# CILAB-MA/gpudrive_lab

Hardware: AMD Instinct MI355X
Metric: agent-steps/sec at 1024 worlds x 64 agents; achieved HBM GB/s on obs kernel (higher is better)
Workload: dtype f32

## Files before the change

gpudrive_lab_amd/csrc/engine.cpp:

```cpp
#include <hip/hip_runtime.h>

#include <algorithm>
#include <cmath>
#include <cstdlib>
#include <cstdio>
#include <cstring>
#include <map>
#include <memory>
#include <stdexcept>
#include <atomic>
#include <exception>
#include <string>
#include <thread>
#include <vector>

#include "dev_mem.hpp"
#include "engine.hpp"
#include "gd_math.hpp"
#include "scene.hpp"
#ifdef GD_CLOCKS
namespace gd { void set_clocks_read(unsigned long long *out); void step_clocks_read(unsigned long long *out); }
#endif
#ifndef GD_GRID_MIN_CELL
#define GD_GRID_MIN_CELL 16.f
// ... 125 lines not shown
    std::vector<gd::DevMem> internal;
    std::vector<std::string> scenes;
    std::vector<int32_t> deleted;
    std::vector<WorldHost> world_host;
    int cu_count = 256;
    Growable<float2, 320, 640> road_xy;
    Growable<Float8, 320, 640> road_aux, road_rec;
    Growable<gd::RoadBox, 0, 64> boxes;
    Growable<int32_t, 0, 64> cell_off, cell_items;
    Growable<float4, 0, 64> cell_hdr;
    Growable<int32_t, 0, 64> rcell_off;
    Growable<uint16_t, 64, 128> rcell_items, rcell_pos;
    Growable<float2, 64, 128> rcell_xy;
    Growable<float4, 0, 64> road_blk;
    int32_t *d_road_off = nullptr, *d_box_off = nullptr, *d_blk_off = nullptr;
    gd::GridHdr *d_grid = nullptr, *d_rgrid = nullptr;
    float4 *d_road_bbox = nullptr;
    float *d_road_rbmax = nullptr;
    static constexpr int kRing = 8;
    PinnedFlags h_flags[kRing];
    Event flag_ev[kRing];
    int ring_pos = 0;
    static constexpr size_t kEvRing = 32;
    Stream side;
    Event ev_fork, ev_join;
    size_t lin_cap = 0;
    int32_t *d_row_of_slot = nullptr, *d_slot_of_row = nullptr, *d_row_count = nullptr;
    int32_t *d_lin_list = nullptr, *d_lin_list_dyn = nullptr;
    bool full_pass_next = false;
    int64_t lin_static_agents = 0;
    int64_t host_skipped = 0;
    bool rk_possible = false;
    bool rk_alloc = false;

    bool ensure_rank_buffers() {
        if (rk_alloc) return true;
        const size_t WA = static_cast<size_t>(W) * A;
        std::vector<gd::DevMem> mine;
        gd::DevSim n = d;
        try {
            alloc_into(mine, n.rk_E, WA * GD_RANK_CAP + 64);
            alloc_into(mine, n.rk_spc, WA * GD_RANK_SPL);
            if (std::getenv("GPUDRIVE_RANK_ALLOC_FAIL") != nullptr)
                throw HipError("GPUDRIVE_RANK_ALLOC_FAIL: simulated allocation failure of the rank replay's buffers");
            alloc_into(mine, n.rk_kt, WA * GD_RANK_KT);
            alloc_into(mine, n.rk_heap, WA * GD_RANK_HEAP_DW);
            alloc_into(mine, n.rk_cpe, WA * GD_RANK_NCP);
            alloc_into(mine, n.rk_n, WA);
            alloc_into(mine, n.rk_fallback, WA / 32);
            alloc_into(mine, n.rk_streak, WA / 32);
            alloc_into(mine, n.cp_road, 2 * WA * GD_RANK_NCP);
            alloc_into(mine, n.cp_T, 2 * WA * GD_RANK_NCP);
            alloc_into(mine, n.cp_hdr, 2 * WA);
            alloc_into(mine, n.rk_words, WA * GD_RANK_NCH);
            alloc_into(mine, n.rk_tl, WA);
            alloc_into(mine, n.rk_hist, 544);
            alloc_into(mine, n.rk_ticket, WA);
            alloc_into(mine, n.rk_order, WA);
            alloc_into(mine, n.rk_list, 8 * WA);
            n.rk_nlong = static_cast<int>(std::max<size_t>(WA / 4, 64));
            alloc_into(mine, n.rk_longlist, n.rk_nlong);
            alloc_into(mine, n.rk_longslot, WA);
            alloc_into(mine, n.rk_E_long, static_cast<size_t>(n.rk_nlong) * GD_RANK_CAP_LONG + 64);
            alloc_into(mine, n.rk_kt_long, static_cast<size_t>(n.rk_nlong) * GD_RANK_KT_LONG);
            internal.reserve(internal.size() + mine.size());
        } catch (const HipError &) {
            (void)hipGetLastError();
            rk_possible = false;
            d.rk_on = 0;
            return false;
        }
        for (gd::DevMem &m : mine) internal.push_back(std::move(m));
        d = n;
        rk_alloc = true;
        return true;
    }
    bool timing = false;
    std::vector<EventPair> ev_pool[gd::KERNEL_TIMED];
    size_t ev_head[gd::KERNEL_TIMED] = {};
    size_t ev_used[gd::KERNEL_TIMED] = {};
    double ev_ms[gd::KERNEL_TIMED] = {};
    int64_t ev_launches[gd::KERNEL_TIMED] = {};

    ~gd_sim() {
        (void)hipDeviceSynchronize();
        if (step_graph) (void)hipGraphExecDestroy(step_graph);
    }

    template <typename T>
    static void alloc_into(std::vector<gd::DevMem> &into, T *&field, size_t count) {
        const size_t bytes = std::max<size_t>(count * sizeof(T), 16);
        into.emplace_back(bytes);
        HIP_CHECK(hipMemset(into.back().get(), 0, bytes));
        field = static_cast<T *>(into.back().get());
    }
    template <typename T>
    T *alloc_internal(size_t count) {
        T *p = nullptr;
        alloc_into(internal, p, count);
        return p;
    }

    void collect_timing(int k, size_t keep = 0) {
        while (ev_used[k] > keep) {
            const EventPair &e = ev_pool[k][ev_head[k]];
            float ms = 0.f;
            if (hipEventSynchronize(e.stop.get()) == hipSuccess && hipEventElapsedTime(&ms, e.start.get(), e.stop.get()) == hipSuccess) {
// ... 2198 lines not shown
```

gpudrive_lab_amd/csrc/engine.hpp:

```cpp
#pragma once
#include <hip/hip_runtime.h>

#include <cstdint>

#include "../../include/gpudrive_amd.h"

#ifndef GD_MAP_OBS_AW
#define GD_MAP_OBS_AW 32
#endif

#define GD_RANK_CAP 1280
#define GD_RANK_NCP 40
#define GD_RANK_HEAP_DW 104
#define GD_RANK_CAP_LONG 2560
#define GD_RANK_KT_LONG 164
#define GD_RH_LONG 537
#define GD_RANK_NCH 320
#define GD_RANK_SPL 256
#define GD_RANK_KT 84
#define GD_RANK_AUDIT 536
#define GD_LIN_BLK 16
#define GD_SKIP_SLOTS 4096

#ifdef GD_DIAG
// ... 49 lines not shown
    const float4 *boxes;
    const GridHdr *grid;
    const int32_t *cell_off;
    const int32_t *cell_items;
    const float4 *cell_hdr;
    const GridHdr *rgrid;
    const int32_t *rcell_off;
    const uint16_t *rcell_items;
    const float2 *rcell_xy;
    const uint16_t *rcell_pos;
    float4 *knn_prev;
    const int32_t *lin_list, *lin_list_dyn;
    int lin_blocks, lin_blocks_dyn;
    int lin_dyn_off;
    const float4 *road_blk;
    const int32_t *blk_off;
    int lin_apw;
    int lin_on;
    uint4 *pose_stamp;
    int pose_skip;
    int32_t *bev_dirty;
    int32_t *bev_list;
    int32_t *bev_count;
    int bev_all_dirty;
    int32_t *lidar_dirty;
    float *lidar_head;
    float *pack;
    int pack_only;
    const int32_t *row_of_slot, *slot_of_row;
    int n_rows;
    int pack_rows;
    unsigned long long *bad_actions;
    unsigned long long *stat_skipped;
    int split_partner;
    int step_dbg;
    int rk_on;
    int rk_max_roads;
    int rk_min_roads;
    int rk_dbg;
    uint16_t *rk_E;
    int rk_nlong;
    int32_t *rk_longlist;
    int32_t *rk_longslot;
    uint16_t *rk_E_long;
    float *rk_kt_long;
    uint16_t *rk_spc;
    float *rk_kt;
    uint32_t *rk_heap;
    uint16_t *rk_cpe;
    int32_t *rk_hist;
    int32_t *rk_ticket;
    int32_t *rk_order;
    int32_t *rk_list;
    uint32_t *rk_words;
    float *rk_tl;
    const float4 *road_bbox;
    const float *road_rbmax;
    int32_t *rk_n;
    int32_t *rk_fallback;
    int32_t *rk_streak;
    uint16_t *cp_road;
    float *cp_T;
    float4 *cp_hdr;
    int warm_k;
    int warm_all;
    int32_t *warm_flags;
    unsigned long long *warm_count;
    const float *pack_weights;
};

void launch_kernel(const DevSim &d, hipStream_t st, int which, bool move);
void launch_map_obs(const DevSim &d, hipStream_t st, bool move);
void launch_map_obs_rank(const DevSim &d, hipStream_t st);
void launch_map_obs_linear(const DevSim &d, hipStream_t st, bool move);
void launch_bev(const DevSim &d, hipStream_t st);
void launch_lidar(const DevSim &d, hipStream_t st);
void launch_pack_obs(const DevSim &d, hipStream_t st, float *out);
void launch_expert_actions(const DevSim &d, hipStream_t st, float *actions, float *pos, float *vel, float *yaw, int *valid);
void launch_set_log_actions(const DevSim &d, hipStream_t st, int t);
void launch_episode_step(const DevSim &d, hipStream_t st, const gd_episode_config &c, const gd_episode_buffers &b);
void launch_draw_weights(const DevSim &d, hipStream_t st, const gd_episode_config &c, const gd_episode_buffers &b,
                         const int32_t *worlds, int n);
void launch_pack_obs_rows(const DevSim &d, hipStream_t st, float *out,
                          const float *weights);
void launch_learner_rows(hipStream_t st, const uint8_t *mask, size_t slots, int32_t *row_of_slot, int32_t *slot_of_row,
                         int32_t *count);
void launch_discrete_actions(const DevSim &d, hipStream_t st, const int64_t *indices, const float *table, int n_actions);
void launch_pack_obs_conditioned(const DevSim &d, hipStream_t st, const float *weights, float *out);
void launch_record(const DevSim &d, hipStream_t st, const gd_record_buffers &b, int t, bool pre);
void launch_bc_rollout_row(const DevSim &d, hipStream_t st, const gd_bc_rollout_buffers &b, int t, int num_stack);
void launch_bc_rollout_actions(const DevSim &d, hipStream_t st, const gd_bc_rollout_buffers &b, int t);
void launch_bc_rollout_post(const DevSim &d, hipStream_t st, const gd_bc_rollout_buffers &b, int t, bool more);
void launch_bc_rollout_summary(hipStream_t st, const gd_bc_rollout_buffers &b);
void launch_policy_rollout_actions(const DevSim &d, hipStream_t st, const gd_policy_rollout_buffers &b, int t);
void launch_policy_rollout_book(const DevSim &d, hipStream_t st, const gd_policy_rollout_buffers &b, int t);
void launch_policy_rollout_finish(const DevSim &d, hipStream_t st, const gd_policy_rollout_buffers &b, int n_steps);
void launch_il_index(const gd_il_dataset &ds, hipStream_t st, int64_t rows, int32_t *counts, int32_t *kept,
                     const int64_t *entry_offset, const int64_t *kept_ordinal, int32_t *entries);
void launch_il_batch(const gd_il_dataset &ds, hipStream_t st, const gd_il_batch_buffers &b,
                     int split);
void launch_il_future(const gd_il_dataset &ds, const gd_il_future &fu, hipStream_t st, const gd_il_future_buffers &b,
                      int split);
void launch_rollout_store(const gd_rollout &ro, hipStream_t st, const float *obs, const float *value, const int64_t *action,
                          const float *logprob, const float *reward, const uint8_t *done, const uint8_t *mask,
                          bool streaming);
void launch_rollout_sort(const gd_rollout &ro, hipStream_t st, const int64_t *offset, int64_t *idxs);
void launch_rollout_gae(const gd_rollout &ro, hipStream_t st, const int64_t *idxs, float gamma, float gae_lambda, float *delta,
// ... 53 lines not shown
```

gpudrive_lab_amd/csrc/map_obs_rank.hip:

```cpp
#include <hip/hip_runtime.h>

#include <algorithm>
#include <type_traits>

#include "engine.hpp"
#include "gd_math.hpp"
#include "rank_heap.hpp"

namespace gd {

namespace {

constexpr int K = GD_MAP_OBS_K;
constexpr int CAP = GD_RANK_CAP;
constexpr int NCP = GD_RANK_NCP;
constexpr int SPL = GD_RANK_SPL;
constexpr int KT = GD_RANK_KT;
constexpr int TILE = 32;
constexpr int CAP_LONG = GD_RANK_CAP_LONG;
template <int CAP_T>
struct RankGeo {
    static constexpr bool LONG = CAP_T > CAP;
    static constexpr int NG = CAP_T / 64;
    static constexpr int NMAX = CAP_T - 8;
    static constexpr int NB = CAP_T;
    static constexpr int NLIN = CAP_T * 3 / 5;
    static constexpr int TSH = LONG ? 6 : 5;
    static constexpr int RSH = LONG ? 4 : 5;
    static constexpr int KTN = LONG ? GD_RANK_KT_LONG : GD_RANK_KT;
};
constexpr int NB = RankGeo<CAP>::NB;
static_assert(K + (NCP - 1) * TILE >= CAP && K + (NCP - 1) * 64 >= CAP_LONG, "a checkpoint slot for every tile of candidates");
static_assert(CAP % 64 == 0 && NB % 128 == 0 && CAP < 2047 && CAP_LONG % 640 == 0 && CAP_LONG < 4095, "geometry; less + 1 fits 11 / 12 bits");
static_assert(SPL >= K + 31 && SPL <= CAP && KT >= CAP / 16 + 1, "every slot the finish looks up; an entry per 16 slots + the last");
constexpr int RK_FAR = 1 << 30;
constexpr int RK_TIES = 1 << 30;

__device__ __forceinline__ void wave_sync() {
    __builtin_amdgcn_fence(__ATOMIC_RELEASE, "wavefront");
    __builtin_amdgcn_wave_barrier();
    __builtin_amdgcn_fence(__ATOMIC_ACQUIRE, "wavefront");
}

__device__ __forceinline__ int wave_incl_scan(int v) {
    v += __builtin_amdgcn_update_dpp(0, v, 0x111, 0xf, 0xf, false);
    v += __builtin_amdgcn_update_dpp(0, v, 0x112, 0xf, 0xf, false);
    v += __builtin_amdgcn_update_dpp(0, v, 0x114, 0xf, 0xf, false);
    v += __builtin_amdgcn_update_dpp(0, v, 0x118, 0xf, 0xf, false);
    v += __builtin_amdgcn_update_dpp(0, v, 0x142, 0xa, 0xf, false);
    v += __builtin_amdgcn_update_dpp(0, v, 0x143, 0xc, 0xf, false);
    return v;
}

#define GD_DPP_SELF(v, ctrl, rows) __builtin_amdgcn_update_dpp((v), (v), (ctrl), (rows), 0xf, false)
__device__ __forceinline__ int wave_max(int v) {
    v = max(v, GD_DPP_SELF(v, 0x111, 0xf));
    v = max(v, GD_DPP_SELF(v, 0x112, 0xf));
    v = max(v, GD_DPP_SELF(v, 0x114, 0xf));
    v = max(v, GD_DPP_SELF(v, 0x118, 0xf));
    v = max(v, GD_DPP_SELF(v, 0x142, 0xa));
    v = max(v, GD_DPP_SELF(v, 0x143, 0xc));
    return __builtin_amdgcn_readlane(v, 63);
}
__device__ __forceinline__ float wave_max_nonneg(float f) { return __int_as_float(wave_max(__float_as_int(f))); }
__device__ __forceinline__ float wave_min_nonneg(float f) { return __int_as_float(~wave_max(~__float_as_int(f))); }
__device__ __forceinline__ int wave_sum(int v) { return __builtin_amdgcn_readlane(wave_incl_scan(v), 63); }

#ifndef GD_NT_SCAN_STORE
#define GD_NT_SCAN_STORE 0
#endif
#ifndef GD_NT_WORDS_LOAD
#define GD_NT_WORDS_LOAD 1
#endif
#ifndef GD_NT_FINISH_LOAD
#define GD_NT_FINISH_LOAD 1
#endif
#ifndef GD_NT_REPLAY_LOAD
#define GD_NT_REPLAY_LOAD 1
#endif
typedef unsigned int u4v __attribute__((ext_vector_type(4)));
typedef unsigned int u2v __attribute__((ext_vector_type(2)));
template <typename T>
__device__ __forceinline__ T stream_load(const T *p) { return __builtin_nontemporal_load(p); }
template <typename T>
__device__ __forceinline__ void stream_store(T v, T *p) { __builtin_nontemporal_store(v, p); }
__device__ __forceinline__ uint4 stream_load(const uint4 *p) {
    const u4v v = __builtin_nontemporal_load(reinterpret_cast<const u4v *>(p));
    return make_uint4(v.x, v.y, v.z, v.w);
}
__device__ __forceinline__ void stream_store(uint4 v, uint4 *p) {
    u4v t; t.x = v.x; t.y = v.y; t.z = v.z; t.w = v.w;
    __builtin_nontemporal_store(t, reinterpret_cast<u4v *>(p));
}
__device__ __forceinline__ uint2 stream_load(const uint2 *p) {
    const u2v v = __builtin_nontemporal_load(reinterpret_cast<const u2v *>(p));
    return make_uint2(v.x, v.y);
}
__device__ __forceinline__ void stream_store(uint2 v, uint2 *p) {
    u2v t; t.x = v.x; t.y = v.y;
    __builtin_nontemporal_store(t, reinterpret_cast<u2v *>(p));
}

__device__ __forceinline__ int audited(const DevSim &d, int idx, int size) {
    if ((unsigned int)idx < (unsigned int)size) return idx;
    atomicAdd(&d.rk_hist[GD_RANK_AUDIT], 1);
    return idx < 0 ? 0 : size - 1;
}

__device__ __forceinline__ bool rank_lt(unsigned int a, unsigned int b, unsigned int tm = 31u) { return (a | tm) < b; }

constexpr int SCAN_TILE = 2048;

template <int A_T>
__global__ __launch_bounds__(256) void k_knn_scan(DevSim d) {
    if (d.gate_any && *d.any_reset == 0) return;
    constexpr int HALVES = A_T / 64;
    const int w = blockIdx.x / HALVES, a0 = (blockIdx.x % HALVES) * 64;
    const int tid = threadIdx.x, wave = tid >> 6, lane = tid & 63;
    const int n = d.shape[w * 2 + 0];
    if (a0 >= n) return;
    const int a = a0 + lane;
    const bool live = a < n;
    const size_t i = (size_t)w * A_T + a;
    const size_t WA = (size_t)d.W * A_T;
    const int r0 = d.road_off[w];
    const int R = d.road_off[w + 1] - r0;

    __shared__ __attribute__((aligned(16))) float2 s_xy[SCAN_TILE];
    __shared__ unsigned short s_first[NCP][64];
    __shared__ float s_thr[NCP][64];
    __shared__ int s_ncp[64];
    __shared__ unsigned int s_needy[2];
    constexpr int TB = 8;
    __shared__ __attribute__((aligned(16))) unsigned int s_tr[4][TB][65];
    static_assert(sizeof(float4) * 64 + sizeof(float) * 192 <= sizeof(unsigned int) * 4 * TB * 65 && 4 * 256 * 4 <= sizeof(float2) * SCAN_TILE, "aliases fit");
    float4 *const s_hdr = reinterpret_cast<float4 *>(&s_tr[0][0][0]);
    float *const s_bx = reinterpret_cast<float *>(s_hdr + 64), *const s_by = s_bx + 64, *const s_bm = s_by + 64;
    unsigned int (*const s_hist)[256] = reinterpret_cast<unsigned int (*)[256]>(s_xy);

    float ex = 0.f, ey = 0.f;
    if (live) { ex = d.px[i]; ey = d.py[i]; }
    unsigned long long ranked = 0ull;
    int list_base = 0;
    if (wave == 0) {
        int ncp = 0;
        float4 h0 = make_float4(0.f, 0.f, __int_as_float(0), 0.f), h1 = h0;
        if (live) { h0 = d.cp_hdr[i]; h1 = d.cp_hdr[WA + i]; }
        s_hdr[lane] = h0;
        wave_sync();
        if (live) {
            const float4 bb = d.road_bbox[w];
            const float ddx = fmaxf(fmaxf(bb.x - ex, ex - bb.z), 0.f), ddy = fmaxf(fmaxf(bb.y - ey, ey - bb.w), 0.f);
            const float far = d.p.observationRadius * 1.01f + 1.f;
            int state = 1, reason = -1;
            if (R >= K && ddx * ddx + ddy * ddy > far * far) {
                state = RK_FAR;
                d.sel_hdr[i * 2] = make_float4(ex, ey, d.qw[i], d.qz[i]);
                d.sel_hdr[i * 2 + 1] = make_float4(__int_as_float(0), __int_as_float(r0), 0.f, 0.f);
                d.cp_hdr[i] = make_float4(ex, ey, __int_as_float(0), 0.f);
            } else {
                const int n0 = __float_as_int(h0.z), n1 = __float_as_int(h1.z);
                const float m0 = n0 > 0 ? sqrtf((ex - h0.x) * (ex - h0.x) + (ey - h0.y) * (ey - h0.y)) : __builtin_inff();
                const float m1 = n1 > 0 ? sqrtf((ex - h1.x) * (ex - h1.x) + (ey - h1.y) * (ey - h1.y)) : __builtin_inff();
                int set = m1 < m0 ? 1 : 0;
                float move = set ? m1 : m0;
                int n_cp = set ? n1 : n0;
                size_t src = i;
                if (move > 6.f) {
                    float best = move;
                    int donor = -1;
                    for (int j = 0; j < 64; j++) {
                        const float4 hj = s_hdr[j];
                        const float dj = __float_as_int(hj.z) > 0 ? sqrtf((ex - hj.x) * (ex - hj.x) + (ey - hj.y) * (ey - hj.y)) : __builtin_inff();
                        if (dj < best) { best = dj; donor = j; }
                    }
                    if (donor >= 0) {
                        move = best;
                        set = 0;
                        n_cp = __float_as_int(s_hdr[donor].z);
                        src = (size_t)w * A_T + a0 + donor;
                    }
                }
                const bool eligible = R >= K && R >= d.rk_min_roads && R <= d.rk_max_roads;
                const int grp = (int)(i / 32);
                const bool bypass = eligible && d.rk_streak[grp] >= 3 && ((d.rk_hist[513] + grp) & 63) != 0;
                const float iw = d.qw[i], iz = d.qz[i];
                const float z2 = iz * iz;
                const float det = (1.f - 2.f * z2) * (1.f - 2.f * z2) + 4.f * z2 * (iw * iw);
                const float margin = 1.00001f / fminf(det, 1.f);
                if (!eligible || bypass) {
                    state = 0;
                    ncp = 0;
                    reason = bypass ? -5 : -2;
                    d.rk_fallback[i / 32] = 1;
                } else if (n_cp <= 0 || move > 6.f) {
                    ncp = -1;
                    s_bx[lane] = ex; s_by[lane] = ey; s_bm[lane] = margin;
                } else {
                    ncp = n_cp;
                    const unsigned short *cr = d.cp_road + ((size_t)set * WA + src) * NCP;
                    const float *ct = d.cp_T + ((size_t)set * WA + src) * NCP;
                    float t = 1.f;
                    for (int q = 0; q < ncp; q++) {
                        t = ct[q];
                        const float reach = sqrtf(t) * 1.0001f + move * 1.0001f + 1e-3f;
                        float thr = reach * reach * 1.0001f * margin;
                        if (!(thr >= 0.f)) thr = __builtin_inff();
                        s_first[q][lane] = cr[q];
                        s_thr[q][lane] = thr;
                    }
                    d.rk_tl[i] = t;
                }
            }
            d.rk_n[i] = state;
            d.rk_ticket[i] = reason;
            if (state == RK_FAR) ncp = 0;
        }
        s_ncp[lane] = ncp;
        {
            const unsigned long long nd = __ballot(ncp < 0);
            if (lane == 0) { s_needy[0] = (unsigned int)nd; s_needy[1] = (unsigned int)(nd >> 32); }
        }
        if (ncp < 0) ncp = 1;
        ranked = __ballot(ncp > 0);
    }
    __syncthreads();
    {
        const unsigned long long needy = (unsigned long long)s_needy[0] | (unsigned long long)s_needy[1] << 32;
        if (needy != 0ull) {
            constexpr int BASE = (127 - 2) << 4;
            unsigned int *hist = s_hist[wave];
            int turn = 0;
            for (unsigned long long rest = needy; rest != 0ull; rest &= rest - 1ull, turn++) {
                if ((turn & 3) != wave) continue;
                const int al = __ffsll((long long)rest) - 1;
                const float bx = s_bx[al], by = s_by[al], mg = s_bm[al];
#pragma unroll
                for (int k = 0; k < 4; k++) hist[k * 64 + lane] = 0u;
                if (lane == 0) { s_first[0][al] = (unsigned short)((K / 32) * 32); s_thr[0][al] = __builtin_inff(); }
                const float ratio = exp2f(log2f(fmaxf((float)R / 256.f, 1.f)) / (float)(NCP - 2));
                float pf = 256.f, tlast = __builtin_inff();
                int pq = 256, q = 1;
                float2 nxt = lane < R ? d.road_xy[r0 + lane] : make_float2(0.f, 0.f);
                for (int rb = 0; rb < R; rb += 64) {
                    const float2 xy = nxt;
                    if (rb + 64 + lane < R) nxt = d.road_xy[r0 + rb + 64 + lane];
                    if (rb + lane < R) {
                        const float dx = xy.x - bx, dy = xy.y - by;
                        const float d2 = __builtin_fmaf(dx, dx, dy * dy);
                        atomicAdd(&hist[min(255, max(0, (int)(__float_as_uint(d2) >> 19) - BASE))], 1u);
                    }
                    if (rb + 64 == pq && q < NCP && pq < R) {
                        wave_sync();
                        const uint4 h = reinterpret_cast<const uint4 *>(hist)[lane];
                        const int own = (int)(h.x + h.y + h.z + h.w);
                        const int incl = wave_incl_scan(own), excl = incl - own;
                        int jb = 0, before = excl;
                        if (before + (int)h.x < K) { before += (int)h.x; jb = 1;
                            if (before + (int)h.y < K) { before += (int)h.y; jb = 2;
                                if (before + (int)h.z < K) { jb = 3; } } }
                        const unsigned long long cross = __ballot(excl < K && incl >= K);
                        const int Lc = __ffsll((long long)cross) - 1;
                        const int bucket = 4 * Lc + __builtin_amdgcn_readlane(jb, Lc);
                        const float T = bucket >= 255 ? __builtin_inff() : __uint_as_float((unsigned int)(bucket + 1 + BASE) << 19);
                        if (lane == 0) {
                            const float reach = sqrtf(T) * 1.0001f + 1e-3f;
                            float thr = reach * reach * 1.0001f * mg * 1.001f;
                            if (!(thr >= 0.f)) thr = __builtin_inff();
                            s_first[q][al] = (unsigned short)min(pq, 65535);
                            s_thr[q][al] = thr;
                        }
                        tlast = T;
                        q++;
                        pf *= ratio;
                        pq = max(pq + 64, ((int)pf + 63) & ~63);
                    }
                }
                if (lane == 0) {
                    s_ncp[al] = q;
                    d.rk_tl[(size_t)w * A_T + a0 + al] = tlast < 1e30f ? tlast : 1.f;
                }
            }
            __syncthreads();
        }
    }
    const int ncp = s_ncp[lane];
    if (__syncthreads_or(ncp > 0 ? 1 : 0) == 0) return;
    int q = -1;
    const int nch = (R + 31) >> 5;
    uint32_t *words = d.rk_words + ((size_t)w * A_T + a0) * GD_RANK_NCH;
    for (int tile = 0; tile < R; tile += SCAN_TILE) {
        __syncthreads();
        for (int r = tile + tid; r < min(R, tile + SCAN_TILE); r += 256) s_xy[r - tile] = d.road_xy[r0 + r];
        __syncthreads();
        if (wave == 0 && ranked != 0ull && lane == 0 && tile + SCAN_TILE >= R)
            list_base = atomicAdd(&d.rk_hist[528 + (blockIdx.x & 7)], __popcll(ranked));
#pragma clang loop unroll(disable)
        for (int c_first = (tile >> 5) + wave * 16; c_first < (tile >> 5) + wave * 16 + 16 && c_first < nch; c_first += TB) {
#pragma clang loop unroll(disable)
            for (int k = 0; k < TB; k++) {
                const int c = c_first + k;
                unsigned int wd = 0;
                if (c < nch) {
                    const int base = c << 5;
                    while (q + 1 < ncp && (int)s_first[q + 1][lane] <= base) q++;
                    const float thr = q >= 0 ? s_thr[q][lane] : __builtin_inff();
                    const float2 *t = s_xy + (base - tile);
#pragma unroll
                    for (int j = 31; j >= 0; j--) {
                        const float2 xy = t[j];
                        const float dx = xy.x - ex, dy = xy.y - ey;
                        const float d2 = __builtin_fmaf(dx, dx, dy * dy);
                        wd = __builtin_amdgcn_alignbit(wd, __float_as_uint(d2 - thr), 31);
                    }
                    if (base < K) wd |= K - base >= 32 ? 0xffffffffu : (1u << (K - base)) - 1u;
                    const int left = R - base;
                    if (left < 32) wd &= (1u << left) - 1u;
                }
                s_tr[wave][k][lane] = wd;
            }
            wave_sync();
#pragma unroll
            for (int it = 0; it < TB; it++) {
                const int ag = it * 8 + (lane >> 3), k = lane & 7;
#if GD_NT_SCAN_STORE
                if (c_first + k < nch && s_ncp[ag] > 0) stream_store(s_tr[wave][k][ag], words + (size_t)ag * GD_RANK_NCH + c_first + k);
#else
                if (c_first + k < nch && s_ncp[ag] > 0) words[(size_t)ag * GD_RANK_NCH + c_first + k] = s_tr[wave][k][ag];
#endif
            }
            wave_sync();
        }
    }
    if (wave == 0 && ranked != 0ull) {
        list_base = __builtin_amdgcn_readfirstlane(list_base);
        if (ncp > 0)
            d.rk_list[(size_t)(blockIdx.x & 7) * WA + audited(d, list_base + __popcll(ranked & ((1ull << lane) - 1ull)), (int)WA)] = (int)i;
    }
}

template <int CAP_T>
struct RankLds {
    union {
        unsigned short cidx[CAP_T];
        struct {
            float skey[CAP_T];
            unsigned short spos[CAP_T];
        } s;
        unsigned short spc[CAP_T];
    };
    unsigned int cnt2[RankGeo<CAP_T>::NB / 2];
};
static_assert(sizeof(RankLds<CAP>) <= 10240 && sizeof(RankLds<CAP_LONG>) <= 20480, "sixteen / eight waves per CU");

constexpr int WPL = GD_RANK_NCH / 64;
struct RankIn {
    int i, state, r0, R, li;
    float ex, ey, iw, iz, t_last;
    unsigned int wd[WPL];
};
template <typename T>
__device__ __forceinline__ T uniform_load(const T *p) {
    return *reinterpret_cast<const __attribute__((address_space(4))) T *>(reinterpret_cast<uintptr_t>(p));
}
template <int A_T>
__device__ __forceinline__ RankIn rank_fetch(const DevSim &d, const int *list, int li, int count, int lane) {
    RankIn in;
    in.li = li;
    in.i = li < count ? uniform_load(list + li) : 0;
    in.state = li < count ? uniform_load(d.rk_n + in.i) : 0;
    const int w = in.i / A_T;
    in.r0 = uniform_load(d.road_off + w);
    in.R = uniform_load(d.road_off + w + 1) - in.r0;
    in.ex = uniform_load(d.px + in.i); in.ey = uniform_load(d.py + in.i);
    in.iw = uniform_load(d.qw + in.i); in.iz = -uniform_load(d.qz + in.i);
    in.t_last = uniform_load(d.rk_tl + in.i);
    const int nch = (in.R + 31) >> 5;
    const uint32_t *words = d.rk_words + (size_t)in.i * GD_RANK_NCH;
#pragma unroll
    for (int k = 0; k < WPL; k++) {
        const int c = k * 64 + lane;
        in.wd[k] = (in.state == 1 && c < nch) ? (GD_NT_WORDS_LOAD ? stream_load(words + c) : words[c]) : 0u;
    }
    return in;
}

#ifdef GD_CLOCKS
struct PhaseClock {
    unsigned int prev, sum[8];
    __device__ __forceinline__ void mark(int n) {
        const unsigned int t = (unsigned int)__builtin_amdgcn_s_memtime();
        sum[n] += t - prev;
        prev = t;
    }
};
#define GD_PHASE(n) clk.mark(n)
#else
struct PhaseClock {};
#define GD_PHASE(n)
#endif
template <int A_T, int CAP_T>
__device__ __forceinline__ void rank_agent(const DevSim &d, const RankIn &in, int lane, RankLds<CAP_T> &L, PhaseClock &clk, int next_entry,
                                           int count, const int *list, RankIn &nxt) {
    using G = RankGeo<CAP_T>;
    constexpr int NB = G::NB, NLIN = G::NLIN, NMAX = G::NMAX;
    constexpr unsigned int TM = (1u << G::RSH) - 1u;
    if (__builtin_amdgcn_readfirstlane(in.state) != 1) {
        nxt = rank_fetch<A_T>(d, list, next_entry, count, lane);
        return;
    }
    auto uni = [](int v) -> int { return __builtin_amdgcn_readfirstlane(v); };
    auto unif = [](float v) -> float { return __int_as_float(__builtin_amdgcn_readfirstlane(__float_as_int(v))); };
    const int i = uni(in.i), r0 = uni(in.r0), R = uni(in.R);
    const int group = i / 32;
    constexpr int NG = G::NG;

    const int nch = (R + 31) >> 5;
    {
        int mine = 0;
#pragma unroll
        for (int k = 0; k < WPL; k++) {
            const int c = k * 64 + lane;
            unsigned int wd = k * 64 < nch ? in.wd[k] : 0u;
            if (k == 0) wd = c < K / 32 ? 0u : (c == K / 32 ? wd & ~((1u << (K % 32)) - 1u) : wd);
            mine += __popc(wd);
        }
        const int total = K + wave_sum(mine);
        if (total > NMAX) {
            if (lane == 0) {
                bool passed_on = false;
                if (!G::LONG && total <= RankGeo<CAP_LONG>::NMAX) {
                    const int slot = atomicAdd(&d.rk_hist[GD_RH_LONG], 1);
                    if (slot < d.rk_nlong) {
                        d.rk_longlist[slot] = i;
                        passed_on = true;
                    }
                }
                if (!passed_on) {
                    d.rk_n[i] = 0;
                    d.rk_ticket[i] = -3;
                    d.rk_fallback[group] = 1;
                }
            }
            nxt = rank_fetch<A_T>(d, list, next_entry, count, lane);
            return;
        }
    }

    static_assert(K == 200 && CAP >= 256, "roads 0..K-1: four stores per lane");
#pragma unroll
    for (int q = 0; q < 4; q++)
        if (q * 64 + lane < K) L.cidx[q * 64 + lane] = (unsigned short)(q * 64 + lane);
    int nin = K;
#pragma unroll
    for (int k = 0; k < WPL; k++) {
        if (k * 64 >= nch) break;
        const int c = k * 64 + lane;
        unsigned int wd = in.wd[k];
        if (k == 0) wd = c < K / 32 ? 0u : (c == K / 32 ? wd & ~((1u << (K % 32)) - 1u) : wd);
        const int pc = __popc(wd);
#ifdef GD_CLOCKS
        clk.sum[7] += (unsigned int)wave_max(pc) << 8;
#endif
        const int incl = wave_incl_scan(pc);
        int pos = nin + incl - pc;
        nin += __builtin_amdgcn_readlane(incl, 63);
        while (wd) {
            L.cidx[pos++] = (unsigned short)((c << 5) + __ffs(wd) - 1);
            wd &= wd - 1u;
        }
    }
    wave_sync();
    const int bin = 255 - min(255, (nin - K) / 5);
    int ticket = 0;
    if (lane == 0) ticket = bin << 20 | atomicAdd(&d.rk_hist[bin], 1);
    GD_PHASE(1);
    if (GD_DIAG_IS(d.rk_dbg, 1)) {
        nxt = rank_fetch<A_T>(d, list, next_entry, count, lane);
        return;
    }
    if (lane <= (nin - K) >> G::TSH) {
        const int road = (int)L.cidx[K - 1 + (lane << G::TSH)];
        d.cp_road[(size_t)i * NCP + lane] = (unsigned short)(lane ? min(65535, (road + 1 + 31) & ~31) : (K / 32) * 32);
    }
    constexpr int GQ = 5;
    static_assert(NG % GQ == 0, "whole groups");
    int ci[NG];
#pragma unroll
    for (int g0 = 0; g0 < NG; g0 += GQ) {
#pragma unroll
        for (int u = 0; u < GQ; u++) ci[g0 + u] = 0;
        if (g0 * 64 < nin) {
            int v[GQ];
#pragma unroll
            for (int u = 0; u < GQ; u++) v[u] = (int)L.cidx[(g0 + u) * 64 + lane];
#pragma unroll
            for (int u = 0; u < GQ; u++) ci[g0 + u] = (g0 + u) * 64 + lane < nin ? v[u] : 0;
        }
    }
    wave_sync();
    const float ex = unif(in.ex), ey = unif(in.ey), iw = unif(in.iw), iz = unif(in.iz);
    const float kmax = d.radius_key_max;
    const float2 *rxy = d.road_xy + r0;
    float key[NG];
    const float t_last = unif(in.t_last);
    float split = (t_last > 0.f && t_last < 1e30f) ? t_last * 1.5f : 1.f;
    int nle = 0, nlow = 0;
    float kmax_seen = 0.f, kmin_seen = __builtin_inff();
#pragma unroll
    for (int g0 = 0; g0 < NG; g0 += GQ) {
#pragma unroll
        for (int u = 0; u < GQ; u++) key[g0 + u] = 0.f;
        if (g0 * 64 < nin) {
            float2 xy[GQ];
#pragma unroll
            for (int u = 0; u < GQ; u++) xy[u] = rxy[(unsigned int)ci[g0 + u]];
            static_assert(GQ == 5, "operand list");
            asm volatile("" : "+v"(xy[0].x), "+v"(xy[0].y), "+v"(xy[1].x), "+v"(xy[1].y), "+v"(xy[2].x), "+v"(xy[2].y),
                              "+v"(xy[3].x), "+v"(xy[3].y), "+v"(xy[4].x), "+v"(xy[4].y));
#pragma unroll
            for (int u = 0; u < GQ; u++) {
                const int g = g0 + u;
                key[g] = ego_dist2(ex, ey, iw, iz, xy[u].x, xy[u].y);
                const bool on = g * 64 + lane < nin;
                nle += ((on & (key[g] <= kmax)) ? 1 : 0) + ((on & (key[g] < split)) ? 1 << 16 : 0);
                kmax_seen = fmaxf(kmax_seen, on ? key[g] : 0.f);
                kmin_seen = fminf(kmin_seen, on ? key[g] : __builtin_inff());
            }
        }
    }
    nxt = rank_fetch<A_T>(d, list, next_entry, count, lane);
    nle = wave_sum(nle);
    kmax_seen = wave_max_nonneg(kmax_seen);
    kmin_seen = wave_min_nonneg(kmin_seen);
    nlow = nle >> 16;
    nle &= 0xffff;
    GD_PHASE(2);
    if (GD_DIAG_IS(d.rk_dbg, 2)) return;

    for (int b = lane; b < NB / 2; b += 64) L.cnt2[b] = 0u;
    wave_sync();
    const bool jumped = nlow * 4 < nin || nlow == nin;
    const float lin_lo = jumped ? kmin_seen : 0.f;
    const int nlin = jumped ? NB : NLIN;
    const float lin_scale = jumped ? (float)NB / fmaxf(kmax_seen - kmin_seen, 1e-30f) : (float)NLIN / split;
    if (jumped) split = __builtin_inff();
    const unsigned int split_bits = __float_as_uint(split);
    const float log_scale = (float)(NB - NLIN) / (float)(max(__float_as_uint(kmax_seen), split_bits + 1u) - split_bits + 1u);
    auto bucket_of = [&](float k) -> int {
        if (k < split) return min(nlin - 1, max(0, (int)((k - lin_lo) * lin_scale)));
        return NLIN + min(NB - NLIN - 1, (int)((float)(__float_as_uint(k) - split_bits) * log_scale));
    };
#pragma unroll
    for (int g = 0; g < NG; g++) {
        if (g * 64 < nin) {
            const int b = bucket_of(key[g]);
            ci[g] |= b << 16;
            if (g * 64 + lane < nin) atomicAdd(&L.cnt2[b >> 1], 1u << ((b & 1) * 16));
        }
    }
    wave_sync();
    {
        constexpr int WPB = NB / 64 / 2;
        static_assert(WPB * 128 == NB, "whole counter words per lane");
        unsigned int own[WPB];
        int sum = 0;
#pragma unroll
        for (int k = 0; k < WPB; k++) { own[k] = L.cnt2[lane * WPB + k]; sum += (int)(own[k] & 0xffffu) + (int)(own[k] >> 16); }
        int run = wave_incl_scan(sum) - sum;
#pragma unroll
        for (int k = 0; k < WPB; k++) {
            const int lo = run, hi = run + (int)(own[k] & 0xffffu);
            run = hi + (int)(own[k] >> 16);
            L.cnt2[lane * WPB + k] = (unsigned int)lo | (unsigned int)hi << 16;
        }
    }
    wave_sync();
    GD_PHASE(3);
    if (GD_DIAG_IS(d.rk_dbg, 3)) return;
#pragma unroll
    for (int g0 = 0; g0 < NG; g0 += GQ) {
        if (g0 * 64 < nin) {
            int sl[GQ];
#pragma unroll
// ... 111 lines not shown
        if (lane == 0) {
            d.rk_n[i] = 0;
            d.rk_ticket[i] = ticket | RK_TIES;
            d.rk_fallback[group] = 1;
        }
        return;
    }
    unsigned short *const E_row = G::LONG ? d.rk_E_long + (size_t)uni(in.li) * CAP_LONG : d.rk_E + (size_t)i * CAP;
    const unsigned int ulane = (unsigned int)lane;
#pragma unroll
    for (int g = 0; g < NG; g++) {
        if (g * 64 < nin) {
            if (g * 64 + lane < nin) {
                const unsigned int e = (unsigned int)ci[g] >> 16;
                stream_store((unsigned short)e, E_row + (g * 64u + ulane));
                const int slot = (int)(e >> G::RSH) - 1 + (int)(e & TM);
                if (slot < SPL) L.spc[slot] = (unsigned short)(ci[g] & 0xffff);
            }
        }
    }
    wave_sync();
    {
        static_assert(SPL == 256, "four slots per lane");
        const uint2 v = reinterpret_cast<const uint2 *>(L.spc)[lane];
        stream_store(v, reinterpret_cast<uint2 *>(d.rk_spc + (size_t)i * SPL) + ulane);
    }
    if (lane == 0) {
        d.rk_n[i] = nin | (nle << 16) | (has_tie ? 1 << 28 : 0) | (G::LONG ? 1 << 29 : 0);
        if (G::LONG) d.rk_longslot[i] = uni(in.li);
        d.rk_ticket[i] = ticket;
    }
    GD_PHASE(6);
}

template <int A_T, int CAP_T>
__global__ __launch_bounds__(64, CAP_T > CAP ? 2 : 4) void k_knn_rank(DevSim d) {
    if (d.gate_any && *d.any_reset == 0) return;
    __shared__ RankLds<CAP_T> L;
    constexpr bool LONG = RankGeo<CAP_T>::LONG;
    const int stride = LONG ? (int)gridDim.x : (int)(gridDim.x >> 3);
    const int xcd = blockIdx.x & 7;
    const int count = LONG ? min(uniform_load(d.rk_hist + GD_RH_LONG), d.rk_nlong) : uniform_load(d.rk_hist + 528 + xcd);
    const int *list = LONG ? d.rk_longlist : d.rk_list + (size_t)xcd * d.W * A_T;
    int t = LONG ? (int)blockIdx.x : (int)(blockIdx.x >> 3);
    RankIn cur = rank_fetch<A_T>(d, list, t, count, threadIdx.x);
    PhaseClock clk;
#ifdef GD_CLOCKS
    for (int k = 0; k < 8; k++) clk.sum[k] = 0u;
    clk.prev = (unsigned int)__builtin_amdgcn_s_memtime();
#endif
    for (; t < count; t += stride) {
        RankIn nxt;
        GD_PHASE(0);
        rank_agent<A_T, CAP_T>(d, cur, threadIdx.x, L, clk, t + stride, count, list, nxt);
        wave_sync();
        cur = nxt;
    }
#ifdef GD_CLOCKS
    if (threadIdx.x == 0)
        for (int k = 0; k < 8; k++) atomicAdd(reinterpret_cast<unsigned int *>(&d.rk_hist[516 + k]), clk.sum[k] >> 8);
#endif
}

#ifndef GD_RANK_AWR
#define GD_RANK_AWR 64
#endif
constexpr int AWR = GD_RANK_AWR;
typedef unsigned int __attribute__((may_alias)) heap_u32;
typedef unsigned short __attribute__((may_alias)) heap_u16;
struct RankHeap {
    heap_u32 *pr;
    __device__ __forceinline__ unsigned int pair(int j) const { return pr[j * AWR]; }
    __device__ __forceinline__ unsigned int get(int g) const {
        return reinterpret_cast<const heap_u16 *>(pr + (g >> 1) * AWR)[g & 1];
    }
    __device__ __forceinline__ void set(int g, unsigned int v) const {
        reinterpret_cast<heap_u16 *>(pr + (g >> 1) * AWR)[g & 1] = (unsigned short)v;
    }
    __device__ __forceinline__ void set_pair(int j, unsigned int v) const { pr[j * AWR] = v; }
};
static_assert(rank_heap::NPAIR == 128, "s_pair of k_knn_replay");

__global__ __launch_bounds__(256) void k_knn_order(DevSim d) {
    if (d.gate_any && *d.any_reset == 0) return;
    __shared__ int s_part[4];
    __shared__ int s_start[256];
    const int tl = threadIdx.x;
    const int c = d.rk_hist[tl];
    const int incl = wave_incl_scan(c);
    if ((tl & 63) == 63) s_part[tl >> 6] = incl;
    __syncthreads();
    int before = 0;
    for (int k = 0; k < (tl >> 6); k++) before += s_part[k];
    s_start[tl] = before + incl - c;
    if (blockIdx.x == 0 && tl == 255) {
        d.rk_hist[512] = before + incl;
        d.rk_hist[513]++;
        for (int x = 0; x < 8; x++) d.rk_hist[528 + x] = 0;
        d.rk_hist[GD_RH_LONG] = 0;
    }
#ifdef GD_CLOCKS
    if (blockIdx.x == 0) d.rk_hist[256 + tl] = 0;
#endif
    __syncthreads();
    const int t = blockIdx.x * 256 + tl;
    if (t >= d.live_count) return;
    const int i = d.live_list[t];
// ... 368 lines not shown
```

Baseline: 64.24 million.

## Replace per-road candidate bitmask scan with block-culled candidate gathering in rank kernel

The scan kernel no longer computes a per-road bitmask over all roads and writes it to global memory. It stores only compact per-agent checkpoint rows (first road index and threshold). The rank kernel culls road blocks against bounding circles, then tests only roads in surviving blocks and writes candidate indices and keys directly to LDS. This removes the full-road scan and the bitmask round-trip through HBM, at the cost of more per-wave work inside the rank kernel and extra LDS table space.

```diff
diff --git a/gpudrive_lab_amd/csrc/engine.cpp b/gpudrive_lab_amd/csrc/engine.cpp
--- a/gpudrive_lab_amd/csrc/engine.cpp
+++ b/gpudrive_lab_amd/csrc/engine.cpp
@@ -201,7 +201,7 @@
             alloc_into(mine, n.cp_road, 2 * WA * GD_RANK_NCP);
             alloc_into(mine, n.cp_T, 2 * WA * GD_RANK_NCP);
             alloc_into(mine, n.cp_hdr, 2 * WA);
-            alloc_into(mine, n.rk_words, WA * GD_RANK_NCH);
+            alloc_into(mine, n.rk_cp, WA * GD_RANK_NCP);
             alloc_into(mine, n.rk_tl, WA);
             alloc_into(mine, n.rk_hist, 544);
             alloc_into(mine, n.rk_ticket, WA);
diff --git a/gpudrive_lab_amd/csrc/engine.hpp b/gpudrive_lab_amd/csrc/engine.hpp
--- a/gpudrive_lab_amd/csrc/engine.hpp
+++ b/gpudrive_lab_amd/csrc/engine.hpp
@@ -125,7 +125,7 @@
     int32_t *rk_ticket;
     int32_t *rk_order;
     int32_t *rk_list;
-    uint32_t *rk_words;
+    uint2 *rk_cp;
     float *rk_tl;
     const float4 *road_bbox;
     const float *road_rbmax;
diff --git a/gpudrive_lab_amd/csrc/map_obs_rank.hip b/gpudrive_lab_amd/csrc/map_obs_rank.hip
--- a/gpudrive_lab_amd/csrc/map_obs_rank.hip
+++ b/gpudrive_lab_amd/csrc/map_obs_rank.hip
@@ -5,6 +5,7 @@
 
 #include "engine.hpp"
 #include "gd_math.hpp"
+#include "rank_cand.hpp"
 #include "rank_heap.hpp"
 
 namespace gd {
@@ -65,13 +66,10 @@
 __device__ __forceinline__ float wave_max_nonneg(float f) { return __int_as_float(wave_max(__float_as_int(f))); }
 __device__ __forceinline__ float wave_min_nonneg(float f) { return __int_as_float(~wave_max(~__float_as_int(f))); }
 __device__ __forceinline__ int wave_sum(int v) { return __builtin_amdgcn_readlane(wave_incl_scan(v), 63); }
-
-#ifndef GD_NT_SCAN_STORE
-#define GD_NT_SCAN_STORE 0
-#endif
-#ifndef GD_NT_WORDS_LOAD
-#define GD_NT_WORDS_LOAD 1
-#endif
+__device__ __forceinline__ int bits_below_lane(unsigned long long b) {
+    return (int)__builtin_amdgcn_mbcnt_hi((unsigned int)(b >> 32), __builtin_amdgcn_mbcnt_lo((unsigned int)b, 0u));
+}
+
 #ifndef GD_NT_FINISH_LOAD
 #define GD_NT_FINISH_LOAD 1
 #endif
@@ -108,8 +106,6 @@
 }
 
 __device__ __forceinline__ bool rank_lt(unsigned int a, unsigned int b, unsigned int tm = 31u) { return (a | tm) < b; }
-
-constexpr int SCAN_TILE = 2048;
 
 template <int A_T>
 __global__ __launch_bounds__(256) void k_knn_scan(DevSim d) {
@@ -126,17 +122,13 @@
     const int r0 = d.road_off[w];
     const int R = d.road_off[w + 1] - r0;
 
-    __shared__ __attribute__((aligned(16))) float2 s_xy[SCAN_TILE];
     __shared__ unsigned short s_first[NCP][64];
     __shared__ float s_thr[NCP][64];
     __shared__ int s_ncp[64];
     __shared__ unsigned int s_needy[2];
-    constexpr int TB = 8;
-    __shared__ __attribute__((aligned(16))) unsigned int s_tr[4][TB][65];
-    static_assert(sizeof(float4) * 64 + sizeof(float) * 192 <= sizeof(unsigned int) * 4 * TB * 65 && 4 * 256 * 4 <= sizeof(float2) * SCAN_TILE, "aliases fit");
-    float4 *const s_hdr = reinterpret_cast<float4 *>(&s_tr[0][0][0]);
-    float *const s_bx = reinterpret_cast<float *>(s_hdr + 64), *const s_by = s_bx + 64, *const s_bm = s_by + 64;
-    unsigned int (*const s_hist)[256] = reinterpret_cast<unsigned int (*)[256]>(s_xy);
+    __shared__ float4 s_hdr[64];
+    __shared__ float s_bx[64], s_by[64], s_bm[64];
+    __shared__ unsigned int s_hist[4][256];
 
     float ex = 0.f, ey = 0.f;
     if (live) { ex = d.px[i]; ey = d.py[i]; }
@@ -201,12 +193,14 @@
                     const unsigned short *cr = d.cp_road + ((size_t)set * WA + src) * NCP;
                     const float *ct = d.cp_T + ((size_t)set * WA + src) * NCP;
                     float t = 1.f;
+                    unsigned int fmax = 0u;
                     for (int q = 0; q < ncp; q++) {
                         t = ct[q];
                         const float reach = sqrtf(t) * 1.0001f + move * 1.0001f + 1e-3f;
                         float thr = reach * reach * 1.0001f * margin;
                         if (!(thr >= 0.f)) thr = __builtin_inff();
-                        s_first[q][lane] = cr[q];
+                        fmax = rank_cand::running_max(fmax, cr[q]);
+                        s_first[q][lane] = (unsigned short)fmax;
                         s_thr[q][lane] = thr;
                     }
                     d.rk_tl[i] = t;
@@ -223,6 +217,7 @@
         }
         if (ncp < 0) ncp = 1;
         ranked = __ballot(ncp > 0);
+        if (ranked != 0ull && lane == 0) list_base = atomicAdd(&d.rk_hist[528 + (blockIdx.x & 7)], __popcll(ranked));
     }
     __syncthreads();
     {
@@ -286,50 +281,14 @@
     }
     const int ncp = s_ncp[lane];
     if (__syncthreads_or(ncp > 0 ? 1 : 0) == 0) return;
-    int q = -1;
-    const int nch = (R + 31) >> 5;
-    uint32_t *words = d.rk_words + ((size_t)w * A_T + a0) * GD_RANK_NCH;
-    for (int tile = 0; tile < R; tile += SCAN_TILE) {
-        __syncthreads();
-        for (int r = tile + tid; r < min(R, tile + SCAN_TILE); r += 256) s_xy[r - tile] = d.road_xy[r0 + r];
-        __syncthreads();
-        if (wave == 0 && ranked != 0ull && lane == 0 && tile + SCAN_TILE >= R)
-            list_base = atomicAdd(&d.rk_hist[528 + (blockIdx.x & 7)], __popcll(ranked));
-#pragma clang loop unroll(disable)
-        for (int c_first = (tile >> 5) + wave * 16; c_first < (tile >> 5) + wave * 16 + 16 && c_first < nch; c_first += TB) {
-#pragma clang loop unroll(disable)
-            for (int k = 0; k < TB; k++) {
-                const int c = c_first + k;
-                unsigned int wd = 0;
-                if (c < nch) {
-                    const int base = c << 5;
-                    while (q + 1 < ncp && (int)s_first[q + 1][lane] <= base) q++;
-                    const float thr = q >= 0 ? s_thr[q][lane] : __builtin_inff();
-                    const float2 *t = s_xy + (base - tile);
-#pragma unroll
-                    for (int j = 31; j >= 0; j--) {
-                        const float2 xy = t[j];
-                        const float dx = xy.x - ex, dy = xy.y - ey;
-                        const float d2 = __builtin_fmaf(dx, dx, dy * dy);
-                        wd = __builtin_amdgcn_alignbit(wd, __float_as_uint(d2 - thr), 31);
-                    }
-                    if (base < K) wd |= K - base >= 32 ? 0xffffffffu : (1u << (K - base)) - 1u;
-                    const int left = R - base;
-                    if (left < 32) wd &= (1u << left) - 1u;
-                }
-                s_tr[wave][k][lane] = wd;
-            }
-            wave_sync();
-#pragma unroll
-            for (int it = 0; it < TB; it++) {
-                const int ag = it * 8 + (lane >> 3), k = lane & 7;
-#if GD_NT_SCAN_STORE
-                if (c_first + k < nch && s_ncp[ag] > 0) stream_store(s_tr[wave][k][ag], words + (size_t)ag * GD_RANK_NCH + c_first + k);
-#else
-                if (c_first + k < nch && s_ncp[ag] > 0) words[(size_t)ag * GD_RANK_NCH + c_first + k] = s_tr[wave][k][ag];
-#endif
-            }
-            wave_sync();
+    {
+        uint2 *rows = d.rk_cp + ((size_t)w * A_T + a0) * NCP;
+        for (int e = tid; e < 64 * NCP; e += 256) {
+            const int ag = e / NCP, q = e - ag * NCP;
+            const int n_ag = s_ncp[ag];
+            if (n_ag > 0)
+                rows[e] = q < n_ag ? make_uint2((unsigned int)s_first[q][ag], __float_as_uint(s_thr[q][ag]))
+                                   : make_uint2(rank_cand::NO_CP, __float_as_uint(__builtin_inff()));
         }
     }
     if (wave == 0 && ranked != 0ull) {
@@ -342,7 +301,10 @@
 template <int CAP_T>
 struct RankLds {
     union {
-        unsigned short cidx[CAP_T];
+        struct {
+            float ckey[CAP_T];
+            unsigned short cidx[CAP_T];
+        } c;
         struct {
             float skey[CAP_T];
             unsigned short spos[CAP_T];
@@ -352,12 +314,17 @@
     unsigned int cnt2[RankGeo<CAP_T>::NB / 2];
 };
 static_assert(sizeof(RankLds<CAP>) <= 10240 && sizeof(RankLds<CAP_LONG>) <= 20480, "sixteen / eight waves per CU");
-
-constexpr int WPL = GD_RANK_NCH / 64;
+constexpr int LSTN = (GD_MAX_ROAD_ENTITIES + GD_LIN_BLK - 1) / GD_LIN_BLK + 15;
+constexpr int LSTN4 = (LSTN + 3) & ~3;
+static_assert(LSTN4 <= 1024 && NCP < 64 && rank_cand::CHUNK % GD_LIN_BLK == 0 && 64 % GD_LIN_BLK == 0, "block and count share 16 bits; a block inside one chunk; whole blocks per pass");
+constexpr size_t CAND_TABLES = LSTN4 * sizeof(unsigned short) + (NCP + 1) * sizeof(float);
+static_assert(CAND_TABLES <= sizeof(RankLds<CAP>::cnt2) && CAND_TABLES <= sizeof(RankLds<CAP_LONG>::cnt2), "the tables fit the idle counters of both instantiations");
+
 struct RankIn {
-    int i, state, r0, R, li;
+    int i, state, r0, R, b0, li;
     float ex, ey, iw, iz, t_last;
-    unsigned int wd[WPL];
+    unsigned int cfirst;
+    float cthr;
 };
 template <typename T>
 __device__ __forceinline__ T uniform_load(const T *p) {
@@ -375,13 +342,11 @@
     in.ex = uniform_load(d.px + in.i); in.ey = uniform_load(d.py + in.i);
     in.iw = uniform_load(d.qw + in.i); in.iz = -uniform_load(d.qz + in.i);
     in.t_last = uniform_load(d.rk_tl + in.i);
-    const int nch = (in.R + 31) >> 5;
-    const uint32_t *words = d.rk_words + (size_t)in.i * GD_RANK_NCH;
-#pragma unroll
-    for (int k = 0; k < WPL; k++) {
-        const int c = k * 64 + lane;
-        in.wd[k] = (in.state == 1 && c < nch) ? (GD_NT_WORDS_LOAD ? stream_load(words + c) : words[c]) : 0u;
-    }
+    in.b0 = uniform_load(d.blk_off + w);
+    uint2 cp = make_uint2(rank_cand::NO_CP, __float_as_uint(__builtin_inff()));
+    if (in.state == 1 && lane < NCP) cp = stream_load(d.rk_cp + (size_t)in.i * NCP + (unsigned int)lane);
+    in.cfirst = cp.x;
+    in.cthr = __uint_as_float(cp.y);
     return in;
 }
 
@@ -415,17 +380,90 @@
     const int group = i / 32;
     constexpr int NG = G::NG;
 
-    const int nch = (R + 31) >> 5;
+    const float ex = unif(in.ex), ey = unif(in.ey), iw = unif(in.iw), iz = unif(in.iz);
+    unsigned short *const lst = reinterpret_cast<unsigned short *>(L.cnt2);
+    float *const tthr = reinterpret_cast<float *>(L.cnt2) + LSTN4 / 2;
+    const unsigned int cfirst = in.cfirst;
+    if (lane < NCP) tthr[lane + 1] = in.cthr;
+    if (lane == 63) tthr[0] = __builtin_inff();
+    const float creach = rank_cand::block_reach(in.cthr);
+    const int nblk = (R + GD_LIN_BLK - 1) / GD_LIN_BLK;
+    const float4 *blk = d.road_blk + uni(in.b0);
+    int nsv = 0;
+    constexpr int CU = 4;
+#pragma clang loop unroll(disable)
+    for (int b0 = 0; b0 < nblk; b0 += 64 * CU) {
+        float4 c[CU];
+#pragma unroll
+        for (int u = 0; u < CU; u++) c[u] = blk[(unsigned int)min(b0 + u * 64 + lane, nblk - 1)];
+#pragma unroll
+        for (int u = 0; u < CU; u++) {
+            const int bb = b0 + u * 64;
+            if (bb < nblk) {
+                const int b = bb + lane;
+                const unsigned int base = (unsigned int)rank_cand::chunk_base_of_block(b, GD_LIN_BLK);
+                const unsigned int base_lo = (unsigned int)rank_cand::chunk_base_of_block(bb, GD_LIN_BLK);
+                const unsigned int base_hi = (unsigned int)rank_cand::chunk_base_of_block(min(bb + 63, nblk - 1), GD_LIN_BLK);
+                const int nlo = __popcll(__ballot(cfirst <= base_lo)), nhi = __popcll(__ballot(cfirst <= base_hi));
+                int cnt = nlo;
+                for (int q = nlo; q < nhi; q++) cnt += (unsigned int)__builtin_amdgcn_readlane((int)cfirst, q) <= base ? 1 : 0;
+                const float reach = __int_as_float(__builtin_amdgcn_ds_bpermute(((cnt - 1) & 63) << 2, __float_as_int(creach)));
+                const bool sv = b < nblk && rank_cand::block_survives(b, GD_LIN_BLK, K, c[u].x, c[u].y, c[u].z, ex, ey, reach);
+                const unsigned long long m = __ballot(sv);
+                if (sv) lst[audited(d, nsv + bits_below_lane(m), LSTN4)] = (unsigned short)(b | cnt << 10);
+                nsv += __popcll(m);
+            }
+        }
+    }
+    wave_sync();
+    int nin = 0;
     {
-        int mine = 0;
-#pragma unroll
-        for (int k = 0; k < WPL; k++) {
-            const int c = k * 64 + lane;
-            unsigned int wd = k * 64 < nch ? in.wd[k] : 0u;
-            if (k == 0) wd = c < K / 32 ? 0u : (c == K / 32 ? wd & ~((1u << (K % 32)) - 1u) : wd);
-            mine += __popc(wd);
-        }
-        const int total = K + wave_sum(mine);
+        constexpr int BPP = 64 / GD_LIN_BLK, PB = 2;
+        const int np = (nsv + BPP - 1) / BPP;
+        const int sub = lane / GD_LIN_BLK, o = lane % GD_LIN_BLK;
+        const float2 *rxy = d.road_xy + r0;
+        struct Batch { int r[PB]; float thr[PB]; float2 xy[PB]; };
+        auto issue = [&](Batch &bt, int p0) {
+#pragma unroll
+            for (int u = 0; u < PB; u++) {
+                const int e = (p0 + u) * BPP + sub;
+                const unsigned int ent = lst[min(e, LSTN4 - 1)];
+                const bool on = e < nsv;
+                const int r = on ? (int)(ent & 1023u) * GD_LIN_BLK + o : R;
+                bt.r[u] = r;
+                bt.thr[u] = tthr[on ? min((int)(ent >> 10), NCP) : 0];
+                bt.xy[u] = rxy[(unsigned int)min(r, R - 1)];
+            }
+        };
+        auto take = [&](const Batch &bt) {
+#pragma unroll
+            for (int u = 0; u < PB; u++) {
+                const bool cand = rank_cand::is_candidate(bt.r[u], K, R, bt.xy[u].x, bt.xy[u].y, ex, ey, bt.thr[u]);
+                const float key = ego_dist2(ex, ey, iw, iz, bt.xy[u].x, bt.xy[u].y);
+                const unsigned long long m = __ballot(cand);
+                const int pos = nin + bits_below_lane(m);
+                if (cand && pos < CAP_T) {
+                    L.c.cidx[pos] = (unsigned short)bt.r[u];
+                    L.c.ckey[pos] = key;
+                }
+                nin += __popcll(m);
+            }
+        };
+        Batch ba, bb;
+        issue(ba, 0);
+#pragma clang loop unroll(disable)
+        for (int p0 = 0; p0 < np; p0 += 2 * PB) {
+            issue(bb, p0 + PB);
+            take(ba);
+            if (p0 + PB >= np) break;
+            issue(ba, p0 + 2 * PB);
+            take(bb);
+        }
+    }
+    wave_sync();
+    nxt = rank_fetch<A_T>(d, list, next_entry, count, lane);
+    {
+        const int total = nin;
         if (total > NMAX) {
             if (lane == 0) {
                 bool passed_on = false;
@@ -442,66 +480,25 @@
                     d.rk_fallback[group] = 1;
                 }
             }
-            nxt = rank_fetch<A_T>(d, list, next_entry, count, lane);
             return;
         }
     }
-
-    static_assert(K == 200 && CAP >= 256, "roads 0..K-1: four stores per lane");
-#pragma unroll
-    for (int q = 0; q < 4; q++)
-        if (q * 64 + lane < K) L.cidx[q * 64 + lane] = (unsigned short)(q * 64 + lane);
-    int nin = K;
-#pragma unroll
-    for (int k = 0; k < WPL; k++) {
-        if (k * 64 >= nch) break;
-        const int c = k * 64 + lane;
-        unsigned int wd = in.wd[k];
-        if (k == 0) wd = c < K / 32 ? 0u : (c == K / 32 ? wd & ~((1u << (K % 32)) - 1u) : wd);
-        const int pc = __popc(wd);
-#ifdef GD_CLOCKS
-        clk.sum[7] += (unsigned int)wave_max(pc) << 8;
-#endif
-        const int incl = wave_incl_scan(pc);
-        int pos = nin + incl - pc;
-        nin += __builtin_amdgcn_readlane(incl, 63);
-        while (wd) {
-            L.cidx[pos++] = (unsigned short)((c << 5) + __ffs(wd) - 1);
-            wd &= wd - 1u;
-        }
-    }
-    wave_sync();
+#ifdef GD_CLOCKS
+    clk.sum[7] += (unsigned int)((nsv + 3) / 4) << 8;
+#endif
     const int bin = 255 - min(255, (nin - K) / 5);
     int ticket = 0;
     if (lane == 0) ticket = bin << 20 | atomicAdd(&d.rk_hist[bin], 1);
     GD_PHASE(1);
-    if (GD_DIAG_IS(d.rk_dbg, 1)) {
-        nxt = rank_fetch<A_T>(d, list, next_entry, count, lane);
-        return;
-    }
+    if (GD_DIAG_IS(d.rk_dbg, 1)) return;
     if (lane <= (nin - K) >> G::TSH) {
-        const int road = (int)L.cidx[K - 1 + (lane << G::TSH)];
+        const int road = (int)L.c.cidx[K - 1 + (lane << G::TSH)];
         d.cp_road[(size_t)i * NCP + lane] = (unsigned short)(lane ? min(65535, (road + 1 + 31) & ~31) : (K / 32) * 32);
     }
     constexpr int GQ = 5;
     static_assert(NG % GQ == 0, "whole groups");
+    const float kmax = d.radius_key_max;
     int ci[NG];
-#pragma unroll
-    for (int g0 = 0; g0 < NG; g0 += GQ) {
-#pragma unroll
-        for (int u = 0; u < GQ; u++) ci[g0 + u] = 0;
-        if (g0 * 64 < nin) {
-            int v[GQ];
-#pragma unroll
-            for (int u = 0; u < GQ; u++) v[u] = (int)L.cidx[(g0 + u) * 64 + lane];
-#pragma unroll
-            for (int u = 0; u < GQ; u++) ci[g0 + u] = (g0 + u) * 64 + lane < nin ? v[u] : 0;
-        }
-    }
-    wave_sync();
-    const float ex = unif(in.ex), ey = unif(in.ey), iw = unif(in.iw), iz = unif(in.iz);
-    const float kmax = d.radius_key_max;
-    const float2 *rxy = d.road_xy + r0;
     float key[NG];
     const float t_last = unif(in.t_last);
     float split = (t_last > 0.f && t_last < 1e30f) ? t_last * 1.5f : 1.f;
@@ -510,26 +507,30 @@
 #pragma unroll
     for (int g0 = 0; g0 < NG; g0 += GQ) {
 #pragma unroll
-        for (int u = 0; u < GQ; u++) key[g0 + u] = 0.f;
+        for (int u = 0; u < GQ; u++) { ci[g0 + u] = 0; key[g0 + u] = 0.f; }
         if (g0 * 64 < nin) {
-            float2 xy[GQ];
-#pragma unroll
-            for (int u = 0; u < GQ; u++) xy[u] = rxy[(unsigned int)ci[g0 + u]];
+            int v[GQ];
+            float kv[GQ];
+#pragma unroll
+            for (int u = 0; u < GQ; u++) {
+                v[u] = (int)L.c.cidx[(g0 + u) * 64 + lane];
+                kv[u] = L.c.ckey[(g0 + u) * 64 + lane];
+            }
             static_assert(GQ == 5, "operand list");
-            asm volatile("" : "+v"(xy[0].x), "+v"(xy[0].y), "+v"(xy[1].x), "+v"(xy[1].y), "+v"(xy[2].x), "+v"(xy[2].y),
-                              "+v"(xy[3].x), "+v"(xy[3].y), "+v"(xy[4].x), "+v"(xy[4].y));
+            asm volatile("" : "+v"(v[0]), "+v"(v[1]), "+v"(v[2]), "+v"(v[3]), "+v"(v[4]), "+v"(kv[0]), "+v"(kv[1]), "+v"(kv[2]), "+v"(kv[3]), "+v"(kv[4]));
 #pragma unroll
             for (int u = 0; u < GQ; u++) {
                 const int g = g0 + u;
-                key[g] = ego_dist2(ex, ey, iw, iz, xy[u].x, xy[u].y);
                 const bool on = g * 64 + lane < nin;
+                ci[g] = on ? v[u] : 0;
+                key[g] = on ? kv[u] : 0.f;
                 nle += ((on & (key[g] <= kmax)) ? 1 : 0) + ((on & (key[g] < split)) ? 1 << 16 : 0);
-                kmax_seen = fmaxf(kmax_seen, on ? key[g] : 0.f);
+                kmax_seen = fmaxf(kmax_seen, key[g]);
                 kmin_seen = fminf(kmin_seen, on ? key[g] : __builtin_inff());
             }
         }
     }
-    nxt = rank_fetch<A_T>(d, list, next_entry, count, lane);
+    wave_sync();
     nle = wave_sum(nle);
     kmax_seen = wave_max_nonneg(kmax_seen);
     kmin_seen = wave_min_nonneg(kmin_seen);
@@ -747,7 +748,9 @@
     for (; t < count; t += stride) {
         RankIn nxt;
         GD_PHASE(0);
-        rank_agent<A_T, CAP_T>(d, cur, threadIdx.x, L, clk, t + stride, count, list, nxt);
+        int lane_v = threadIdx.x;
+        asm volatile("" : "+v"(lane_v));
+        rank_agent<A_T, CAP_T>(d, cur, lane_v, L, clk, t + stride, count, list, nxt);
         wave_sync();
         cur = nxt;
     }
diff --git a/gpudrive_lab_amd/csrc/rank_cand.hpp b/gpudrive_lab_amd/csrc/rank_cand.hpp
--- /dev/null
+++ b/gpudrive_lab_amd/csrc/rank_cand.hpp
@@ -0,0 +1,48 @@
+#pragma once
+
+#include <cmath>
+
+#if defined(__HIPCC__)
+#define GD_RC_FN __host__ __device__ __forceinline__
+#else
+#define GD_RC_FN inline
+#endif
+
+namespace gd {
+namespace rank_cand {
+
+constexpr int CHUNK = 32;
+constexpr unsigned int NO_CP = 0xffffffffu;
+
+GD_RC_FN unsigned int f32_bits(float f) { return __builtin_bit_cast(unsigned int, f); }
+
+GD_RC_FN bool road_passes(float x, float y, float ex, float ey, float thr) {
+    const float dx = x - ex, dy = y - ey;
+    const float d2 = __builtin_fmaf(dx, dx, dy * dy);
+    return (f32_bits(d2 - thr) >> 31) != 0u;
+}
+GD_RC_FN bool is_candidate(int r, int K, int R, float x, float y, float ex, float ey, float thr) {
+    return r < R && (r < K || road_passes(x, y, ex, ey, thr));
+}
+
+GD_RC_FN int cp_in_force(const unsigned int *first, int ncp, int base) {
+    int q = -1;
+    while (q + 1 < ncp && first[q + 1] <= (unsigned int)base) q++;
+    return q;
+}
+GD_RC_FN unsigned int running_max(unsigned int run, unsigned int first) { return first > run ? first : run; }
+GD_RC_FN int cp_count(const unsigned int *first_max, int n, int base) {
+    int c = 0;
+    for (int q = 0; q < n; q++) c += first_max[q] <= (unsigned int)base ? 1 : 0;
+    return c;
+}
+GD_RC_FN int chunk_base_of_block(int b, int blk) { return (b * blk) & ~(CHUNK - 1); }
+
+GD_RC_FN float block_reach(float thr) { return sqrtf(thr) * 1.00001f; }
+GD_RC_FN bool block_survives(int b, int blk, int K, float cx, float cy, float rad, float ex, float ey, float reach) {
+    const float dx = cx - ex, dy = cy - ey, rr = reach + rad;
+    return b * blk < K || !(dx * dx + dy * dy > rr * rr * 1.00001f);
+}
+
+}
+}
```

Result: faster. 65.41 million (median of 6 runs) (+1.8%).
